# phylovi/libsbn

Hardware: AMD Instinct MI355X
Metric: tree log-likelihoods+gradients/sec (batched) (higher is better)
Workload: dtype f64; 1 GPU; DS1 27 taxa x 934 site patterns x 1000 trees per step over 1 GPU(s), JC69+weibull+4 (K=4), phylo_gradients: logL + branch + site gradients; trees_total=1000, trees_per_gpu=1000, taxa=27, patterns=934, categories=4, parallelism=single GPU

## Files before the change

### libsbn_amd/csrc/kernels_walk3.hip

```cpp
#include <hip/hip_runtime.h>

#include <algorithm>
#include <cmath>
#include <cstdlib>
#include <string>
#include <type_traits>

#include "mi_phylo_device_utils.h"
#include "mi_phylo_kernels.h"
#include "mi_phylo_setup_device.h"

namespace miphylo {
namespace {
using namespace dev;

template <int SHIFT>
__device__ __forceinline__ double row_shr_add(double v) {
  const int lo = __double2loint(v), hi = __double2hiint(v);
  const int slo = __builtin_amdgcn_update_dpp(0, lo, 0x110 + SHIFT, 0xf, 0xf, true);
  const int shi = __builtin_amdgcn_update_dpp(0, hi, 0x110 + SHIFT, 0xf, 0xf, true);
  return v + __hiloint2double(shi, slo);
}
template <int SHIFT>
__device__ __forceinline__ double row_ror_add(double v) {
// ... 1022 lines not shown
        store16_sc1(dst + 48, v4i32{me.gslot[1], me.gslot[2], me.gslot[3], me.pad});
      }
    }
  }
  asm volatile("s_waitcnt lgkmcnt(0)" ::: "memory");
  if (ok) {
    if (q == 0) {
      double* dst = reinterpret_cast<double*>(f.ms.models + t);
      const double* src = reinterpret_cast<const double*>(md);
      static_assert(sizeof(DevModel) % 16 == 0, "whole 16-byte pieces");
      for (int i = lane; i < (int)(sizeof(DevModel) / 16); i += 64) store16_sc1(dst + 2 * i, src[2 * i], src[2 * i + 1]);
    }
    const int idx = q * per_q + lane;
    const int node = idx / K, k = idx - node * K;
    const bool live = lane < per_q && node < N - 1;
    if (live) {
      double bl;
      if (!a.rooted) {
        bl = node < N - 2 ? a.bl[(size_t)t * (N - 1) + node] : 0.0;
      } else {
        bl = a.bl[(size_t)t * N + node];
        if (a.rates) bl *= a.rates[(size_t)t * (N - 1) + node];
      }
      const bool tip = node < n;
      lut_record(*md, md->cat_rate[k] * bl, tip, stage + lane * 41);
      const int slot = slot_of[node], m = slot / 6, pos = slot - m * 6;
      const int rec8 = (int)((((size_t)t * max_macros(n) + m) * 6 + pos) * (kPos / 8));
      rec_of[lane] = rec8 + k * (tip ? (int)(kTipCat / 8) : 32);
      len_of[lane] = tip ? 40 : 32;
    } else {
      rec_of[lane] = -1;
      len_of[lane] = 0;
    }
    asm volatile("s_waitcnt lgkmcnt(0)" ::: "memory");
    XSTAMP(st3);
    {
      int rec[8], len[8];
      double va[24], vb[24];
      const int part = lane & 7;
#pragma unroll
      for (int x8 = 0; x8 < 8; x8++) {
        const int th = (lane >> 3) + 8 * x8;
        rec[x8] = rec_of[th];
        len[x8] = len_of[th];
        const int row = min(th, per_q - 1) * 41;
#pragma unroll
        for (int p3 = 0; p3 < 3; p3++) {
          const int d = 2 * (p3 * 8 + part);
          va[3 * x8 + p3] = stage[row + min(d, 38)];
          vb[3 * x8 + p3] = stage[row + min(d, 38) + 1];
        }
      }
#pragma unroll
      for (int i = 0; i < 24; i++) asm volatile("" : "+v"(va[i]), "+v"(vb[i]));
#pragma unroll
      for (int x8 = 0; x8 < 8; x8++)
#pragma unroll
        for (int p3 = 0; p3 < 3; p3++) {
          const int d = 2 * (p3 * 8 + part);
          if (rec[x8] >= 0 && d < len[x8])
            store16_sc1(f.mmats + (size_t)rec[x8] + d, va[3 * x8 + p3], vb[3 * x8 + p3]);
        }
    }
  }
  XSTAMP(st4);
  asm volatile("s_waitcnt vmcnt(0)" ::: "memory");
  XSTAMP(st5);
#ifdef W3_SETUP_STAMPS
  if (lane == 0 && (t == 0 || t == 60 || t == 124) && q < 2)
    printf("setup role t %d q %d: start %lld end %lld model %lld tree %lld records %lld stores issued %lld landed %lld (10 ns ticks)\n", t, q, st0, (long long)__builtin_amdgcn_s_memrealtime(),
           st1 - st0, st2 - st1, st3 - st2, st4 - st3, st5 - st4);
#endif
  if (f.fence == 2) __builtin_amdgcn_fence(__ATOMIC_RELEASE, "agent");
  if (lane == 0 && f.ready && !(f.debug_skip == t + 1 && q == 1))
    __hip_atomic_fetch_add(f.ready + (size_t)t * kReadyStride, kReadyQuarter + (q == 0 ? M : 0), __ATOMIC_RELAXED,
                           __HIP_MEMORY_SCOPE_AGENT);
}

__global__ __launch_bounds__(kTile) void setup_records_kernel(FusedSetupArgs f) {
  extern __shared__ double wlds[];
  fused_setup_role(f, blockIdx.x, reinterpret_cast<char*>(wlds));
}

template <bool RESCALE, int KP>
__global__ __launch_bounds__(kTile, kRegs == 2 ? 3 : 2) void gradient_walk_lut_fused_kernel(LikArgs a, FusedSetupArgs f) {
  extern __shared__ double wlds[];
  if ((int)blockIdx.x < f.setup_blocks) {
    fused_setup_role(f, blockIdx.x, reinterpret_cast<char*>(wlds));
    return;
  }
  walk_lut_body<RESCALE, true, false, KP>(a, wlds, (int)blockIdx.x - f.setup_blocks, f.ready, f.spin_ticks, f.fence);
#ifdef W3_SETUP_STAMPS
  if (threadIdx.x == 0 && (((int)blockIdx.x - f.setup_blocks) % 1499) == 0)
    printf("walk block %d: out %lld\n", (int)blockIdx.x - f.setup_blocks, (long long)__builtin_amdgcn_s_memrealtime());
#endif
}

}

size_t gradient_walk_lut_mats_bytes_per_eval(int n) { return (size_t)max_macros(n) * kVisit; }

static int lut_kp(int K) { return K == 1 ? 1 : (K == 2 ? 2 : 4); }

bool gradient_walk_lut_fused_applies(int n, int K) {
  return gradient_walk_lut_applies(K) && 2 * n - 1 <= 64 && ((2 * n - 2) * K + 3) / 4 <= 64;
}

template <bool RESCALE, int KP>
static void launch_fused_variant(const LikArgs& a, const FusedSetupArgs& f, dim3 grid, size_t lds, hipStream_t s) {
  allow_large_lds(reinterpret_cast<const void*>(gradient_walk_lut_fused_kernel<RESCALE, KP>), lds);
  hipLaunchKernelGGL((gradient_walk_lut_fused_kernel<RESCALE, KP>), grid, dim3(kTile), lds, s, a, f);
}
void launch_gradient_walk_lut_fused(const LikArgs& a_in, const FusedSetupArgs& f_in, int count, bool rescale,
                                    hipStream_t s) {
  if (count <= 0) return;
  LikArgs a = a_in;
  FusedSetupArgs f = f_in;
  a.kp = lut_kp(a.K);
  a.cat_groups = 1;
  a.walk_evals = count;
  f.setup_blocks = kSetupQuarters * count;
  f.xcd_base = f.setup_blocks & 7;
  if (f.spin_ticks <= 0) f.spin_ticks = 100 * 1000 * 1000;
  const int gtiles = gradient_mfma_tiles(a.P, a.K);
  const dim3 grid((unsigned)((size_t)count * gtiles + f.setup_blocks));
  const size_t lds = std::max<size_t>(gradient_walk_lds_bytes(a.n, a.K, rescale, false), fused_setup_lds(a.n, a.K));
  switch ((rescale ? 8 : 0) | a.kp) {
    case 1: launch_fused_variant<false, 1>(a, f, grid, lds, s); break;
    case 2: launch_fused_variant<false, 2>(a, f, grid, lds, s); break;
    case 4: launch_fused_variant<false, 4>(a, f, grid, lds, s); break;
    case 9: launch_fused_variant<true, 1>(a, f, grid, lds, s); break;
    case 10: launch_fused_variant<true, 2>(a, f, grid, lds, s); break;
    default: launch_fused_variant<true, 4>(a, f, grid, lds, s); break;
  }
}

void launch_setup_records(const FusedSetupArgs& f_in, int count, hipStream_t s) {
  if (count <= 0) return;
  FusedSetupArgs f = f_in;
  f.setup_blocks = kSetupQuarters * count;
  f.xcd_base = 0;
  f.ready = nullptr;
  f.fence = 0;
  f.debug_skip = 0;
  const size_t lds = fused_setup_lds(f.ts.n, f.ms.K);
  allow_large_lds(reinterpret_cast<const void*>(setup_records_kernel), lds);
  hipLaunchKernelGGL(setup_records_kernel, dim3((unsigned)f.setup_blocks), dim3(kTile), lds, s, f);
}

void launch_transition_lut(const TransitionMacroArgs& a, hipStream_t s) {
  if (a.count <= 0) return;
  const int per_eval = (a.N - 1) * a.K;
  const dim3 grid(a.count, (per_eval + kTlBlock - 1) / kTlBlock);
  hipLaunchKernelGGL(transition_lut_kernel, grid, dim3(kTlBlock), sizeof(int) * (size_t)(a.N - 1), s, a);
}

bool gradient_walk_lut_applies(int K) { return K >= 1 && K <= 4 && kRegs >= 2; }

template <bool RESCALE, bool ARENA, int KP, int RR>
static void launch_lut_variant(const LikArgs& a, dim3 grid, size_t lds, hipStream_t s, bool resident,
                               int forced) {
  if (ARENA && (forced < 0 ? (a.g_tiles * RR <= 48 * kRegs || resident) : forced != 0)) {
    allow_large_lds(reinterpret_cast<const void*>(gradient_walk_lut_kernel<RESCALE, ARENA, KP, ARENA, RR>), lds);
    hipLaunchKernelGGL((gradient_walk_lut_kernel<RESCALE, ARENA, KP, ARENA, RR>), grid, dim3(kTile), lds, s, a);
    return;
  }
  allow_large_lds(reinterpret_cast<const void*>(gradient_walk_lut_kernel<RESCALE, ARENA, KP, false, RR>), lds);
  hipLaunchKernelGGL((gradient_walk_lut_kernel<RESCALE, ARENA, KP, false, RR>), grid, dim3(kTile), lds, s, a);
}
template <bool ARENA, int RR = kRegs>
static void launch_lut_store(const LikArgs& a, dim3 grid, size_t lds, bool rescale, hipStream_t s,
                             int arena_nt, bool resident = false) {
  switch ((rescale ? 8 : 0) | a.kp) {
    case 1: launch_lut_variant<false, ARENA, 1, RR>(a, grid, lds, s, resident, arena_nt); break;
    case 2: launch_lut_variant<false, ARENA, 2, RR>(a, grid, lds, s, resident, arena_nt); break;
    case 4: launch_lut_variant<false, ARENA, 4, RR>(a, grid, lds, s, resident, arena_nt); break;
    case 9: launch_lut_variant<true, ARENA, 1, RR>(a, grid, lds, s, resident, arena_nt); break;
    case 10: launch_lut_variant<true, ARENA, 2, RR>(a, grid, lds, s, resident, arena_nt); break;
    default: launch_lut_variant<true, ARENA, 4, RR>(a, grid, lds, s, resident, arena_nt); break;
  }
}

void launch_gradient_walk_lut(const LikArgs& a_in, int count, bool rescale, const Switches& sw, hipStream_t s) {
  if (count <= 0) return;
  LikArgs a = a_in;
  a.kp = lut_kp(a.K);
  a.cat_groups = 1;
  a.walk_evals = count;
  const bool wide = kRegs < kRegsWide && a.tile_regs == kRegsWide;
  const int regs = wide ? kRegsWide : kRegs;
  const int gtiles = gradient_mfma_tiles(a.P, a.K, regs);
  const bool arena_variant =
      a.store ? a.store == 2
              : gradient_walk_use_arena(sw.gradient_store, a.n, a.K, rescale, false, (size_t)gtiles * (size_t)count, true, regs);
  const dim3 grid((unsigned)((size_t)count * gtiles));
  if (arena_variant) {
    const int usual = gradient_arena_slots_usual(a.n), sure = gradient_arena_slots_sure(a.n);
    auto lds_for = [&](int slots) { return gradient_walk_lds_bytes_for(a.n, a.K, rescale, false, slots, regs); };
    auto launch = [&](int slots, bool resident) {
      if (wide) launch_lut_store<true, kRegsWide>(a, grid, lds_for(slots), rescale, s, sw.arena_nt, resident);
      else launch_lut_store<true>(a, grid, lds_for(slots), rescale, s, sw.arena_nt, resident);
    };
    a.lds_lo = -1;
    if (arena_single_launch(lds_for(sure), grid.x)) {
      a.lds_slots = sure;
      launch(sure, true);
      return;
    }
    a.lds_slots = usual;
    const bool resident = arena_single_launch(lds_for(usual), grid.x);
    launch(usual, resident);
    if (sure > usual) {
      a.lds_lo = usual;
      a.lds_slots = sure;
      launch(sure, resident);
    }
    return;
  }
  if (wide) {
    const size_t lds = gradient_walk_lds_bytes(a.n, a.K, rescale, false, regs);
    auto go = [&](auto kernel) {
      allow_large_lds(reinterpret_cast<const void*>(kernel), lds);
      hipLaunchKernelGGL(kernel, grid, dim3(kTile), lds, s, a);
    };
    switch ((rescale ? 8 : 0) | a.kp) {
      case 1: go(gradient_walk_lut_kernel<false, false, 1, false, kRegsWide, 1>); break;
      case 2: go(gradient_walk_lut_kernel<false, false, 2, false, kRegsWide, 1>); break;
      case 4: go(gradient_walk_lut_kernel<false, false, 4, false, kRegsWide, 1>); break;
      case 9: go(gradient_walk_lut_kernel<true, false, 1, false, kRegsWide, 1>); break;
      case 10: go(gradient_walk_lut_kernel<true, false, 2, false, kRegsWide, 1>); break;
// ... 38 lines not shown
```

### libsbn_amd/csrc/mi_phylo_call.cpp

```cpp
#include "mi_phylo_engine.h"

namespace {

bool use_arena(const mi_engine* e, bool rescale, bool subst, size_t waves = (size_t)-1, int regs = 0) {
  const bool lut = walk3_possible(e) && e->sw.walk3_arena && !subst && gradient_mfma_groups(e->K) == 1;
  return gradient_walk_use_arena(e->sw.gradient_store, e->n, e->K, rescale, subst, waves, lut, regs);
}
bool walk_fits(const mi_engine* e, bool rescale) { return gradient_walk_fits(e->n, e->K, rescale); }

const char* loglik_kernel_of(const mi_engine* e, bool rescaling) {
  LikArgs probe{};
  probe.n = e->n;
  probe.K = e->K;
  probe.tip_masks = e->have_tip_masks ? e->tip_masks.as<uint8_t>() : nullptr;
  return loglik_kernel_name(probe, rescaling, e->max_slots, e->sw);
}
bool matrix_core_gradient(const mi_engine* e, bool rescaling, bool loglik_is_valu) {
  return !e->sw.hbm_gradient && e->have_tip_masks && walk_fits(e, rescaling) &&
         reduce_tiles_fits(e->N) && (gradient_mfma_groups(e->K) == 1 || !loglik_is_valu);
}

size_t plv_bytes_per_eval(const mi_engine* e) {
  return (size_t)(e->n - 1) * e->K * e->tiles * kTile * 4 * sizeof(double);
}
// ... 38 lines not shown
  const int n = e->n;
  const bool gradient = kind == kGradientCall;
  p.kind = kind;
  p.T = T;
  p.rescaling = rescaling;
  p.rooted = rooted;
  p.gtr = e->spec.subst_model == MI_SUBST_GTR;
  p.groups = 1;
  p.models_per_tree = 1;
  p.E = p.M = T;
  p.mmats_bytes_per_eval = std::max(gradient_walk_mats_bytes_per_eval(n, e->K),
                                    walk3_possible(e) ? gradient_walk_lut_mats_bytes_per_eval(n) : 0);
  p.dominant = loglik_kernel_of(e, rescaling);
  p.loglik_is_valu = std::string(p.dominant) == "loglik_onchip_kernel";
  if (kind == kHessianCall) {
    p.Eg = T;
    p.mfma = !e->sw.hbm_gradient && e->have_tip_masks && e->K <= 4 && walk_fits(e, rescaling);
    p.g_tiles = p.mfma ? gradient_mfma_tiles(e->P, e->K) : e->tiles;
    const size_t waves = (size_t)(route_T ? route_T : T) * gradient_mfma_tiles(e->P, e->K);
    const bool arena = p.mfma && gradient_walk_use_arena(e->sw.gradient_store, n, e->K, rescaling, false, waves, false, 0);
    p.store = !p.mfma ? kStoreHbm : arena ? kStoreArena : kStoreLds;
    p.reserve_arena = arena;
    p.need_slots = !p.mfma;
    p.dominant = p.mfma ? gradient_walk_hess_kernel_name() : gradient_hessian_kernel_name();
    return p;
  }
  if (kind == kNniCall) {
    p.Eg = T;
    p.g_tiles = e->tiles;
    p.store = kStoreHbm;
    p.dominant = nni_scan_kernel_name();
    return p;
  }
  if (kind == kAncestralCall) {
    p.Eg = T;
    p.g_tiles = e->tiles;
    p.store = kStoreHbm;
    p.dominant = ancestral_kernel_name();
    return p;
  }
  if (kind == kPlacementCall) {
    p.Eg = T;
    p.g_tiles = e->tiles;
    p.store = kStoreHbm;
    p.dominant = placement_kernel_name();
    return p;
  }
  if (kind == kSprCall) {
    p.Eg = T;
    p.g_tiles = e->tiles;
    p.store = kStoreHbm;
    p.dominant = spr_kernel_name();
    return p;
  }
  p.mfma = gradient && matrix_core_gradient(e, rescaling, p.loglik_is_valu);
  if (p.mfma) p.groups = gradient_mfma_groups(e->K);
  p.analytic = e->sw.analytic_subst && p.mfma && p.gtr;
  p.tile_regs = p.mfma && !p.analytic && p.groups == 1 ? e->tile_regs : 0;
  p.g_tiles = p.mfma ? gradient_mfma_tiles(e->P, e->K, p.tile_regs) * p.groups : e->tiles;
  p.light = gradient && p.mfma && !p.analytic && p.gtr && !want_subst && !want_site;
  const bool fd = gradient && p.gtr && !p.analytic && !p.light;
  p.site_fused = gradient && e->K > 1 && !fd;
  p.site_separate = gradient && e->K > 1 && fd;
  p.models_per_tree = fd ? kFdModels : 1;
  p.M = T * p.models_per_tree;
  p.Eg = gradient ? T : 0;
  if (fd) p.E += 16 * T;
  if (p.site_separate) {
    p.E += T;
    p.Eg += T;
  }
  p.need_slots = !(gradient && p.mfma && p.groups == 1 && (!p.gtr || p.analytic || p.light));
  const bool arena = p.mfma && use_arena(e, rescaling, p.analytic, (size_t)T * (size_t)p.g_tiles, p.tile_regs);
  p.store = !p.mfma ? kStoreHbm : arena ? kStoreArena : kStoreLds;
  p.reserve_arena = p.mfma && (e->tile_regs || use_arena(e, false, true) || use_arena(e, true, true) ||
                               use_arena(e, false, false) || use_arena(e, true, false));
  p.hand_off_words = gradient && e->fused_setup && walk3_possible(e);
  const bool fuse_possible = p.mfma && walk3_possible(e) && !p.analytic && p.groups == 1 && !arena && !p.tile_regs && e->fused_setup &&
                             e->sw.fuse_finalize && p.E == T && p.models_per_tree == 1 && !p.need_slots &&
                             T <= e->sw.fused_max_trees && gradient_walk_lut_fused_applies(n, e->K);
  p.walk3 = p.mfma && walk3_possible(e) && !p.analytic && p.groups == 1 &&
            (p.tile_regs || (arena ? e->sw.walk3_arena : (e->K > 1 || e->sw.walk3_k1_lds || fuse_possible)));
  p.fuse_setup = p.walk3 && fuse_possible;
  p.setup_records = p.walk3 && !p.fuse_setup && !arena && !p.tile_regs && !p.analytic && p.groups == 1 && e->fused_setup &&
                    p.E == T && p.models_per_tree == 1 && !p.need_slots && T <= kMaxEvals &&
                    gradient_walk_lut_fused_applies(n, e->K) && e->sw.setup_records;
  p.fd_pass = gradient && p.gtr && !p.analytic && want_subst;
  p.site_pass = p.site_separate && want_site;
  p.loglik_runs = !gradient || p.fd_pass || (p.mfma && p.groups > 1);
  p.need_tip_tables = p.loglik_runs && p.loglik_is_valu;
  if (gradient)
    p.dominant = p.fuse_setup ? gradient_walk_lut_fused_kernel_name()
                 : p.walk3    ? gradient_walk_lut_kernel_name()
                 : p.mfma     ? gradient_walk_kernel_name()
                              : gradient_kernel_name();
  return p;
}

std::string plan_path(const mi_engine* e, const CallPlan& p) {
  std::string path = p.dominant;
  if (p.kind != kLogLikCall)
    path += p.store == kStoreHbm ? " store=hbm" : (p.store == kStoreArena ? " store=arena" : " store=lds");
  path += p.fuse_setup ? " setup=in-walk" : (p.setup_records ? " setup=with-records" : " setup=own-launch");
  if (p.kind == kHessianCall) path += " hess";
  if (p.kind == kNniCall) path += " nni";
  if (p.kind == kAncestralCall) path += " ancestral";
  if (p.kind == kPlacementCall) path += " placement";
  if (p.kind == kSprCall) path += " spr";
  if (p.pattern_ll) path += " pattern_ll";
  if (p.tile_regs > kLlR) path += " tile=wide";
  if (p.fd_pass) path += " fd=16";
  if (p.site_pass) path += " site-pass";
  if (p.light) path += " light";
  if (p.analytic) path += " analytic";
  if (p.rescaling) path += " rescaled";
  if (p.rooted) path += " rooted";
  return path + " K=" + std::to_string(e->K);
}

int reserve(mi_engine* e, const CallPlan& p) {
  const int n = e->n, N = e->N, T = p.T;
  const bool gradient = p.kind == kGradientCall;
  if (e->tree_scratch.ensure(sizeof(int32_t) * (size_t)T * 13 * N)) return 1;
  if (e->sched.ensure(sizeof(SchedEntry) * (size_t)T * (n - 1))) return 1;
  if (e->macros.ensure(sizeof(MacroEntry) * (size_t)T * macro_stride(n))) return 1;
  if (e->macro_count.ensure(sizeof(int32_t) * (size_t)T)) return 1;
  if (e->bl_eff.ensure(sizeof(double) * (size_t)T * N)) return 1;
  if (e->models.ensure(sizeof(DevModel) * (size_t)p.M)) return 1;
  if (e->mats.ensure(sizeof(double) * (size_t)p.E * (N - 1) * e->K * 16)) return 1;
  if (e->tip_tables.ensure(sizeof(double) * (size_t)p.E * n * e->K * 20)) return 1;
  if (gradient) {
    if (e->mmats.ensure(p.mmats_bytes_per_eval * (size_t)p.Eg)) return 1;
    if (p.analytic && e->mphi.ensure(p.mmats_bytes_per_eval / 2 * (size_t)p.Eg)) return 1;
  }
  if (p.analytic && e->x_sum.ensure(sizeof(double) * (size_t)p.Eg * kSubstExtra)) return 1;
  if (e->ll_part.ensure(sizeof(double) * (size_t)p.E * e->ll_stride)) return 1;
  if (e->fin_scratch.ensure(sizeof(double) * (size_t)T * 6 * n)) return 1;
  if (e->status.ensure(sizeof(int32_t) * kStatusWords)) return 1;
  if (p.hand_off_words && e->ready.bytes < sizeof(int32_t) * kReadyStride * (size_t)T) {
    if (e->ready.ensure(sizeof(int32_t) * kReadyStride * (size_t)T)) return 1;
    HIP_TRY(hipMemset(e->ready.ptr, 0, e->ready.bytes));
    HIP_TRY(hipDeviceSynchronize());
  }
  if (e->ll_sum.ensure(sizeof(double) * (size_t)p.E)) return 1;
  if (p.kind == kLogLikCall && !p.rooted && e->pattern_ll_out.ensure(sizeof(double) * (size_t)T)) return 1;
  if (gradient && e->g_sum.ensure(sizeof(double) * (size_t)p.Eg * 2 * N)) return 1;
  if (gradient) {
    const size_t per = plv_bytes_per_eval(e);
    const size_t chunk = std::max<size_t>(1, std::min<size_t>(p.Eg, e->plv_budget / per));
    if (!p.mfma && e->plv.ensure(per * chunk)) return 1;
    if (p.reserve_arena) {
      const size_t aper = gradient_arena_bytes_per_eval(n, e->P, e->K);
      const size_t achunk = std::max<size_t>(1, std::min<size_t>(p.Eg, e->plv_budget / aper));
      if (e->plv.ensure(aper * achunk)) return 1;
      if (e->arena_macros.ensure(sizeof(MacroEntry) * (size_t)T * macro_stride(n))) return 1;
      if (e->slot_need.ensure(sizeof(int32_t) * (size_t)T)) return 1;
    }
    const size_t g_width = std::max<size_t>(2 * (size_t)N, (size_t)gradient_mfma_width(n, true));
    if (e->g_part.ensure(sizeof(double) * (size_t)p.Eg * e->ll_stride * gradient_mfma_groups(e->K) *
                         g_width))
      return 1;
    if (e->site_lik.ensure(sizeof(double) * (size_t)p.Eg * e->tiles * kTile)) return 1;
    if (e->site_exp.ensure(sizeof(int32_t) * (size_t)p.Eg * e->tiles * kTile)) return 1;
  }
  return 0;
}


TreeSetupArgs tree_setup_args(const mi_engine* e, const DeviceCall& d, const CallPlan& p) {
  TreeSetupArgs ts{};
  ts.n = e->n;
  ts.T = d.T;
  ts.rooted = d.rooted;
  ts.parent_ids = d.parent_ids;
  ts.bl = d.bl;
  ts.rates = (d.rooted && (d.gradient || d.with_jacobian)) ? d.rates : nullptr;
  ts.scratch = e->tree_scratch.as<int32_t>();
  ts.sched = e->sched.as<SchedEntry>();
  ts.macros = p.mfma ? e->macros.as<MacroEntry>() : nullptr;
  ts.macro_count = e->macro_count.as<int32_t>();
  ts.bl_eff = e->bl_eff.as<double>();
  ts.status = e->status.as<int32_t>();
  ts.max_slots = e->max_slots;
  ts.need_slots = p.need_slots;
  ts.arena_macros = p.store == kStoreArena ? e->arena_macros.as<MacroEntry>() : nullptr;
  ts.slot_need = e->slot_need.as<int32_t>();
// ... 113 lines not shown
  la.map = EvalMap{d.T, p.models_per_tree};
  la.models = e->models.as<DevModel>();
  la.sched = e->sched.as<SchedEntry>();
  la.macros = walk_macros(e, p);
  la.macro_count = e->macro_count.as<int32_t>();
  la.mats = e->mats.as<double>();
  la.mmats = e->mmats.as<double>();
  la.tip_states = e->tip_states.as<int8_t>();
  la.tip_masks = e->have_tip_masks ? e->tip_masks.as<uint8_t>() : nullptr;
  la.tip_partials = e->spec.use_tip_states ? nullptr : e->tip_partials.as<double>();
  la.weights = e->weights.as<double>();
  la.ll_part = e->ll_part.as<double>();
  la.plv = e->plv.as<double>();
  la.g_part = e->g_part.as<double>();
  la.status = e->status.as<int32_t>();
  la.slot_need = e->slot_need.as<int32_t>();
  la.store = p.store;
  if (p.kind == kAncestralCall) {
    la.anc_state = d.out_anc_state;
    la.anc_map = d.out_anc_map;
    la.anc_cat = d.out_anc_cat;
    la.anc_rate = d.out_anc_rate;
    la.anc_tip = d.out_anc_tip;
    return la;
  }
  if (p.kind == kPlacementCall) {
    la.place_half = e->place_half.as<double>();
    la.place_pend = e->place_pend.as<double>();
    la.place_table = e->place_table.as<double>();
    la.place_G = d.G;
    return la;
  }
  if (p.kind == kHessianCall || p.kind == kNniCall || p.kind == kSprCall) return la;
  la.tip_tables = e->tip_tables.as<double>();
  la.mphi = e->mphi.as<double>();
  la.tip_code_tiles = e->have_tip_codes && e->tip_code_tiles.ptr && e->sw.tip_tiles && e->tile_regs == p.tile_regs
                          ? e->tip_code_tiles.as<uint8_t>() : nullptr;
  la.tip_tiles = e->have_tip_masks && e->tip_tiles.ptr && e->sw.tip_tiles ? e->tip_tiles.as<uint8_t>() : nullptr;
  la.tip_codes = e->have_tip_codes ? e->tip_codes.as<uint8_t>() : nullptr;
  la.tile_regs = p.tile_regs;
  la.pattern_ll = p.pattern_ll ? d.out_pattern_ll : nullptr;
  la.pattern_blank = e->pattern_blank.as<uint8_t>();
  return la;
}

void macro_slots(const mi_engine* e, int T, hipStream_t s) {
  launch_macro_slots(e->macros.as<MacroEntry>(), e->arena_macros.as<MacroEntry>(),
                     e->macro_count.as<int32_t>(), e->n, T, e->slot_need.as<int32_t>(),
                     e->status.as<int32_t>(), e->sw, s);
}

void note_call(mi_engine* e, const CallPlan& p, int first_launch_evals, int walk_launches) {
  e->dominant = p.dominant;
  e->last_path = plan_path(e, p);
  e->prof_first_launch_evals = first_launch_evals;
  e->last_evals = p.E;
  e->last_grad_evals = p.Eg;
  e->last_walk_launches = walk_launches;
}

int check_call(const mi_engine* e, const DeviceCall& d, const void* output) {
  if (d.T <= 0) return fail("tree_count must be positive");
  if (!d.parent_ids || !d.bl || !output) return fail("null tree / output pointer");
  if (e->param_count > 0 && !d.params) return fail("null parameter matrix");
  return 0;
}

}

int run_device(mi_engine* e, hipStream_t s, const DeviceCall& d_in) {
  HIP_TRY(hipSetDevice(e->spec.device));
  if (e->s == kAa) return d_in.out_pattern_ll ? fail(kPatternLl4State) : aa_run_device(e, s, d_in);
  if (check_call(e, d_in, d_in.out_pattern_ll ? d_in.out_pattern_ll : d_in.out_ll)) return 1;
  const CallPlan p = plan_call(e, d_in.gradient ? kGradientCall : kLogLikCall, d_in);
  if (reserve(e, p)) return 1;
  DeviceCall d = d_in;
  if (!d.out_ll) d.out_ll = e->pattern_ll_out.as<double>();
  const int n = e->n, N = e->N, T = d.T;
  const bool prof = e->prof_used < e->prof_capacity;
  const bool marks = prof && e->prof_phases;
  PROF_MARK(e, marks, 0, s);

  if (p.setup_records) launch_setup_records(fused_setup_args(e, d, p), T, s);
  const bool slots_done = !p.fuse_setup && !p.setup_records &&
                          launch_setup(tree_setup_args(e, d, p), model_setup_args(e, d, p), e->sw, s);
  if (p.store == kStoreArena && !slots_done) macro_slots(e, T, s);

  TransitionArgs tr = transition_args(e, d, p);
  if (p.mfma && p.groups == 1) {
    if (p.fd_pass) {
      tr.eval_base = T;
      tr.E = 16 * T;
      launch_transition(tr, s);
    }
  } else {
    launch_transition(tr, s);
  }
  auto macro_matrices = [&](int eval_begin, int grad_begin, int count) {
    const TransitionMacroArgs tm = transition_macro_args(e, d, p, eval_begin, grad_begin, count);
    if (p.walk3) launch_transition_lut(tm, s);
    else launch_transition_macro(tm, s);
  };
  if (p.mfma && !p.fuse_setup && !p.setup_records) {
    macro_matrices(0, 0, T);
    if (p.site_pass) macro_matrices(17 * T, T, T);
  }

  const LikArgs la = lik_args(e, d, p);
  int walk_launches = 0;
  auto loglik_range = [&](int eval_begin, int count) {
    launch_in_parts(e, count, 0, walk_launches, [&](int done, int part) {
      LikArgs l = la;
      l.eval_offset = eval_begin + done;
      launch_loglik(l, part, d.rescaling, e->max_slots, e->sw, s);
    });
  };
  auto grad_range = [&](int eval_begin, int grad_begin, int count) {
    launch_in_parts(e, count, vector_bytes_per_eval(e, p), walk_launches, [&](int done, int part) {
      LikArgs g = la;
      g.eval_offset = eval_begin + done;
      g.grad_offset = grad_begin + done;
      if (!p.mfma) return launch_gradient_hbm(g, part, d.rescaling, s);
      if (p.groups > 1) {
        g.site_lik = e->site_lik.as<double>();
        g.site_exp = e->site_exp.as<int32_t>();
        launch_loglik(g, part, d.rescaling, e->max_slots, e->sw, s);
      }
      if (p.fuse_setup) launch_gradient_walk_lut_fused(g, fused_setup_args(e, d, p), part, d.rescaling, s);
      else if (p.walk3) launch_gradient_walk_lut(g, part, d.rescaling, e->sw, s);
      else launch_gradient_walk(g, part, d.rescaling, p.analytic, e->sw, s);
    });
  };
  if (prof) HIP_TRY(hipEventRecord(prof_event(e, 0), s));
  PROF_MARK(e, marks, 1, s);
  PROF_MARK(e, marks, 2, s);
  if (!d.gradient) {
    loglik_range(0, T);
    if (prof) HIP_TRY(hipEventRecord(prof_event(e, 1), s));
    PROF_MARK(e, marks, 3, s);
  } else {
    grad_range(0, 0, T);
    if (prof) HIP_TRY(hipEventRecord(prof_event(e, 1), s));
    PROF_MARK(e, marks, 3, s);
    if (p.fd_pass) loglik_range(T, 16 * T);
    if (p.site_pass) grad_range(17 * T, T, T);
  }
  note_call(e, p, T, walk_launches);

  FinalizeArgs fa = finalize_args(e, d);
  fa.ll_tiles = e->ll_stride;
  fa.g_tiles = p.g_tiles;
  fa.ll_part = e->ll_part.as<double>();
  fa.g_part = e->g_part.as<double>();
  const int ll_kernel_count = p.loglik_is_valu ? e->tiles : loglik_mfma_tiles(e->P, e->K);
  const int grad_kernel_count =
      p.mfma ? (p.groups > 1 ? ll_kernel_count : p.g_tiles) : e->tiles;
  LlCounts ll_used{d.gradient ? grad_kernel_count : ll_kernel_count, ll_kernel_count, 0, 0};
  if (d.gradient && p.gtr && !p.analytic && !p.light) {
    ll_used.mid_lo = T;
    ll_used.mid_hi = 17 * T;
  }
  fa.ll_used = ll_used;
  bool fused = false;
  ReduceArgs ra{};
  if (reduce_tiles_fits(N)) {
    ra.N = N;
    ra.E = p.E;
    ra.Eg = p.Eg;
    ra.ll_tiles = e->ll_stride;
    ra.ll_used = ll_used;
    ra.g_tiles = p.g_tiles;
    ra.ll_part = e->ll_part.as<double>();
    ra.g_part = e->g_part.as<double>();
    ra.ll_sum = e->ll_sum.as<double>();
    ra.g_sum = e->g_sum.as<double>();
    ra.g_width = p.mfma ? gradient_mfma_width(n, p.analytic) : 0;
    ra.extra = p.analytic ? kSubstExtra : 0;
    ra.x_sum = e->x_sum.as<double>();
    ra.n = n;
    ra.T = T;
    ra.macros = walk_macros(e, p);
    ra.macro_count = e->macro_count.as<int32_t>();
    fused = e->sw.fuse_finalize && p.E == T;
    if (!fused) launch_reduce_tiles(ra, s);
    fa.ll_tiles = 1;
    fa.ll_used = LlCounts{1, 1, 0, 0};
// ... 405 lines not shown
```

### libsbn_amd/csrc/mi_phylo_engine.h

```cpp
#pragma once
#include <hip/hip_runtime.h>

#include <algorithm>
#include <cstring>
#include <functional>
#include <string>
#include <vector>

#include "../../include/mi_phylo.h"
#include "mi_phylo_host_arrays.h"
#include "mi_phylo_kernels.h"

namespace miphylo {
int fail(const std::string& msg);
void set_last_error(const std::string& msg);
}
using miphylo::fail;
using namespace miphylo;

#define HIP_TRY(expr)                                                              \
  do {                                                                             \
    hipError_t err__ = (expr);                                                     \
    if (err__ != hipSuccess)                                                       \
      return fail(std::string("HIP error: ") + hipGetErrorString(err__) + " at " + \
// ... 118 lines not shown
  int fused_fallbacks = 0;
  Buffer aa_model, aa_matP, aa_matPT, aa_tipP, aa_tipPQ, aa_exp_cum, aa_exp_loc,
      aa_root_val, aa_root_exp, aa_root_scale;
  bool aa_reserved_gradient = false;
  PinnedArena pinned;
  Switches sw;
  int tile_regs = 0;
  std::vector<mi_engine*> shards;
  int shard_mode = 0;
  std::vector<double> shard_sums;
  Buffer red_ll, red_g, red_site, red_sort;
  long red_ws_entries = -1;
  int red_ws_bits = 0;
  size_t red_ws_bytes = 0;
  Buffer in_pack, out_pack;
  Buffer opt_ws;
  int32_t* opt_word = nullptr;
  Buffer nni_apply_ws;
  Buffer nni_search_ws;
  Buffer pattern_blank;
  Buffer pattern_ll_out;
  Buffer rell_ws;
  Buffer rell_s;
  Buffer dist_codes;
  Buffer dist_model;
  Buffer dist_counts;
  Buffer dist_matrix;
  Buffer nj_ws;
  Buffer place_bl;
  Buffer place_half;
  Buffer place_pend;
  Buffer place_table;
  Buffer spr_bl;
  Buffer spr_half;
  Buffer spr_ws;
  Buffer spr_path;
  Buffer spr_apply_ws;
  Buffer spr_search_ws;
  Buffer split_ws;
  Buffer split_store;
  Buffer split_sort;
  Buffer rf_ws;
  size_t plv_budget = (size_t)8 << 30;
  std::vector<hipEvent_t> prof_events;
  int prof_capacity = 0, prof_used = 0;
  bool prof_phases = false;
  int prof_first_launch_evals = 0;
  const char* dominant = "";
  std::string last_path;
  int64_t last_evals = 0, last_grad_evals = 0;
  int status_tree_offset = 0;
  int last_walk_launches = 1;
  int aa_backoffs = 0;
};


constexpr int kProfEvents = 7;
inline hipEvent_t prof_event(mi_engine* e, int which) {
  return e->prof_events[(size_t)kProfEvents * e->prof_used + which];
}
#define PROF_MARK(e, on, which, s)                                   \
  do {                                                               \
    if (on) HIP_TRY(hipEventRecord(prof_event(e, 2 + (which)), s)); \
  } while (0)

enum CallKind { kLogLikCall, kGradientCall, kHessianCall, kNniCall, kAncestralCall, kPlacementCall, kSprCall };
enum WalkStore { kStoreHbm = 0, kStoreLds = 1, kStoreArena = 2 };
struct CallPlan {
  CallKind kind;
  int T;
  bool rescaling, rooted;
  int E, Eg, M, models_per_tree;
  bool gtr, site_fused, site_separate;
  bool mfma;
  bool walk3;
  WalkStore store;
  int groups;
  int tile_regs;
  int g_tiles;
  bool analytic;
  bool light;
  bool fuse_setup;
  bool setup_records;
  bool need_slots;
  bool fd_pass, site_pass;
  bool loglik_runs;
  bool loglik_is_valu;
  bool pattern_ll;
  bool need_tip_tables;
  size_t mmats_bytes_per_eval;
  bool reserve_arena;
  bool hand_off_words;
  const char* dominant;
};
struct DeviceCall {
  bool gradient = false, rooted = false, with_jacobian = false, rescaling = false;
  int T = 0;
  const int32_t* parent_ids = nullptr;
  const double* bl = nullptr;
  const double* params = nullptr;
  const double* rates = nullptr;
  const int32_t* rate_counts = nullptr;
  const double* heights = nullptr;
  const double* bounds = nullptr;
  const double* ratios = nullptr;
  double* out_ll = nullptr;
  double* out_branch = nullptr;
  double* out_ratios = nullptr;
  double* out_clock = nullptr;
  double* out_site = nullptr;
  double* out_subst = nullptr;
  double* out_hess = nullptr;
  double* out_gsq = nullptr;
  double* out_nni = nullptr;
  int32_t* out_best = nullptr;
  double* out_pattern_ll = nullptr;
  double* out_anc_state = nullptr;
  int8_t* out_anc_map = nullptr;
  double* out_anc_cat = nullptr;
  double* out_anc_rate = nullptr;
  double* out_anc_tip = nullptr;
  int Q = 0, C = 0, G = 0;
  const int8_t* query_states = nullptr;
  const int32_t* column_pattern = nullptr;
  const double* column_weights = nullptr;
  const double* pendant_lengths = nullptr;
  double* out_place_edge_ll = nullptr;
  int8_t* out_place_pendant = nullptr;
  int32_t* out_place_best = nullptr;
  double* out_place_lwr = nullptr;
  double* out_place_tables = nullptr;
  int spr_radius = 0;
  int32_t* out_spr_target = nullptr;
  double* out_spr_delta = nullptr;
  int32_t* out_spr_move = nullptr;
  double* out_spr_table = nullptr;
  int route_T = 0;
};
CallPlan plan_call(const mi_engine* e, CallKind kind, int T, bool rescaling, int route_T = 0,
                   bool rooted = false, bool want_site = true, bool want_subst = true);
inline CallPlan plan_call(const mi_engine* e, CallKind kind, const DeviceCall& d) {
  CallPlan p = plan_call(e, kind, d.T, d.rescaling, d.route_T, d.rooted, d.out_site != nullptr, d.out_subst != nullptr);
  p.pattern_ll = kind == kLogLikCall && d.out_pattern_ll != nullptr;
  return p;
}
std::string plan_path(const mi_engine* e, const CallPlan& p);
bool walk3_possible(const mi_engine* e);
int engine_tile_regs(const mi_engine* e);
int reserve(mi_engine* e, const CallPlan& p);
int reserve_hessian(mi_engine* e, const CallPlan& p);
int reserve_hessian_calls(mi_engine* e, int T);
TreeSetupArgs tree_setup_args(const mi_engine* e, const DeviceCall& d, const CallPlan& p);
ModelSetupArgs model_setup_args(const mi_engine* e, const DeviceCall& d, const CallPlan& p);
FinalizeArgs finalize_args(const mi_engine* e, const DeviceCall& d);
int run_device(mi_engine* e, hipStream_t s, const DeviceCall& d);
int run_hessian_device(mi_engine* e, hipStream_t s, const DeviceCall& d);
int reserve_nni_calls(mi_engine* e, int T);
int run_nni_device(mi_engine* e, hipStream_t s, const DeviceCall& d);
int reserve_ancestral_calls(mi_engine* e, int T);
int run_ancestral_device(mi_engine* e, hipStream_t s, const DeviceCall& d);
int check_placement_shape(const mi_engine* e, int Q, int C, int G);
int reserve_placement_calls(mi_engine* e, int T, int G);
int run_placement_device(mi_engine* e, hipStream_t s, const DeviceCall& d);
int check_spr_shape(const mi_engine* e, int radius);
int reserve_spr_calls(mi_engine* e, int T);
int run_spr_device(mi_engine* e, hipStream_t s, const DeviceCall& d);
// ... 102 lines not shown
```

### libsbn_amd/csrc/mi_phylo_kernels.h

```cpp
#pragma once
#include <hip/hip_runtime.h>

#include "mi_phylo_device.h"
#include "mi_phylo_switches.h"

namespace miphylo {

struct EvalMap {
  int T;
  int models_per_tree;
  __host__ __device__ void decode(int e, int& tree, int& model) const {
    if (e < T) {
      tree = e;
      model = e * models_per_tree;
    } else if (e < 17 * T) {
      tree = (e - T) / 16;
      model = tree * kFdModels + 1 + (e - T) % 16;
    } else {
      tree = e - 17 * T;
      model = tree * kFdModels + 16;
    }
  }
};

// ... 446 lines not shown
}
struct SplitArgs {
  int n, T, W, capacity;
  int hash_bits;
  uint32_t slots;
  const int32_t* parent_ids;
  const double* bl;
  const double* weights;
  int32_t* status;
  uint32_t* store;
  uint32_t* occ_bits;
  uint64_t* occ_hash;
  int32_t* occ_slot;
  void* scan_tmp;
  size_t scan_tmp_bytes;
  int32_t* slot_owner;
  int32_t* slot_first;
  int32_t* slot_trees;
  uint32_t *keys, *vals, *keys2, *vals2;
  void* sort_tmp;
  size_t sort_tmp_bytes;
  int32_t* out_index;
  int32_t* out_count;
  uint32_t* out_bits;
  int32_t* out_first;
  int32_t* out_trees;
  double* out_stats;
};
size_t split_scan_tmp_bytes(size_t occurrences);
size_t split_sort_tmp_bytes(size_t occurrences);
int launch_split_index(const SplitArgs& a, hipStream_t s);
struct RfArgs {
  int n, T;
  const int32_t* split_index;
  const double* bl;
  int32_t* sorted_index;
  double* sorted_length;
  int32_t* sorted_count;
  int32_t* out_rf;
  double* out_bs;
};
void launch_rf(const RfArgs& a, hipStream_t s);
int gradient_mfma_groups(int K);
int gradient_mfma_width(int n, bool subst = false);
void launch_macro_slots(const MacroEntry* macros_in, MacroEntry* macros_out,
                        const int32_t* macro_count, int n, int T, int32_t* need, int32_t* status,
                        const Switches& sw, hipStream_t s);
size_t gradient_arena_bytes_per_eval(int n, int P, int K);
int device_compute_units();
bool arena_single_launch(size_t lds_bytes, size_t waves);
int gradient_arena_slots_sure(int n);
int gradient_arena_slots_usual(int n);
void launch_transition_macro(const TransitionMacroArgs& a, hipStream_t s);
void launch_gradient_walk(const LikArgs& a, int count, bool rescale, bool subst, const Switches& sw, hipStream_t s);
bool gradient_walk_fits(int n, int K, bool rescale);
bool gradient_walk_use_arena(int store, int n, int K, bool rescale, bool subst, size_t waves = (size_t)-1,
                             bool lut = false, int regs = 0);
bool gradient_walk_batches_take_arena(int n, int K, bool lut);
size_t gradient_walk_lds_bytes(int n, int K, bool rescale, bool subst, int regs = 0);
size_t gradient_walk_lds_bytes_for(int n, int K, bool rescale, bool subst, int slots, int regs = 0);
size_t gradient_walk_mats_bytes_per_eval(int n, int K);
const char* gradient_walk_kernel_name();
size_t gradient_walk_lut_mats_bytes_per_eval(int n);
void launch_transition_lut(const TransitionMacroArgs& a, hipStream_t s);
bool gradient_walk_lut_applies(int K);
void launch_gradient_walk_lut(const LikArgs& a, int count, bool rescale, const Switches& sw, hipStream_t s);
constexpr int kReadyStride = 32;
struct FusedSetupArgs {
  TreeSetupArgs ts;
  ModelSetupArgs ms;
  double* mmats;
  int32_t* ready;
  int setup_blocks;
  int spin_ticks;
  int debug_skip;
  int fence;
  int colocate;
  int xcd_base;
};
bool gradient_walk_lut_fused_applies(int n, int K);
void launch_gradient_walk_lut_fused(const LikArgs& a, const FusedSetupArgs& f, int count, bool rescale,
                                    hipStream_t s);
void launch_setup_records(const FusedSetupArgs& f, int count, hipStream_t s);
const char* gradient_walk_lut_kernel_name();
const char* gradient_walk_lut_fused_kernel_name();
int gradient_walk_waves_per_cu(int store, int n, int K);
struct ReduceArgs {
  int N, E, Eg, ll_tiles, g_tiles;
  LlCounts ll_used;
  const double* ll_part;
  const double* g_part;
  double* ll_sum;
  double* g_sum;
  int g_width, n, T;
  const MacroEntry* macros;
  const int32_t* macro_count;
  int extra;
  double* x_sum;
  int keep_offset;
};

struct SubstGradArgs {
  int T, param_count, rates_off, freqs_off;
  const double* params;
  const DevModel* models;
  const double* x_sum;
  double* out_subst;
};
void launch_subst_gradient(const SubstGradArgs& a, hipStream_t s);
constexpr int kSubstExtra = 68;
struct ViReduceArgs {
  int T, N, index_count;
  const double* ll;
  const double* branch;
  const double* site;
  const int32_t* branch_index;
  const double* tree_weights;
  double* out_sums;
  double* out_index_gradient;
};
size_t vi_reduce_workspace_bytes(long entries, int index_count);
int launch_vi_reduce(const ViReduceArgs& a, void* workspace, size_t workspace_bytes, hipStream_t s);
bool reduce_tiles_fits(int N);
void launch_reduce_tiles(const ReduceArgs& a, hipStream_t s);
void launch_finalize(const FinalizeArgs& a, hipStream_t s);
void launch_reduce_finalize(const ReduceArgs& ra, const FinalizeArgs& fa, hipStream_t s);

constexpr int kAa = 20;
constexpr int kAaTile = 16;
constexpr int kAaTipSlack = 512;
constexpr int kAaTileDoubles = 320;
constexpr int kAaPack = 512;
constexpr int kAaPackRows16 = 320;
constexpr int kAaTipTable = 21 * 20;
constexpr int kAaPreTiles = 2;

struct AaModel {
  double pi[kAa];
  double lambda[kAa];
  double Q[kAa * kAa];
  double V[kAa * kAa];
  double Vinv[kAa * kAa];
  double Qpack[kAaPack];
};

struct AaTransitionArgs {
  int n, N, K;
  int eval_offset, evals;
  int gradient;
  const AaModel* model;
  const DevModel* models;
  const double* bl_eff;
  double* matP;
  double* matPT;
  double* tipP;
  double* tipPQ;
};

struct AaWalkArgs {
  int n, N, P, K;
  int tiles;
  int eval_offset, evals;
  int gradient;
  int slots;
  int ring_slots;
  int pre_ring_slots;
// ... 42 lines not shown
```

### libsbn_amd/csrc/mi_phylo_switches.cpp

```cpp
#include "mi_phylo_switches.h"

#include <cerrno>
#include <climits>
#include <cstdlib>
#include <cstring>

namespace miphylo {
namespace {

struct Reader {
  std::string error;

  const char* get(const char* name) {
    const char* v = getenv(name);
    return v && *v ? v : nullptr;
  }
  void reject(const char* name, const char* value, const std::string& expected) {
    if (error.empty()) error = std::string(name) + "=" + value + ": expected " + expected;
  }
  int choice(const char* name, const char* values, int dflt) {
    const char* v = get(name);
    if (!v) return dflt;
    const size_t len = strlen(v);
    int index = 0;
    for (const char* w = values;; index++) {
      const char* end = strchr(w, '|');
      const size_t wlen = end ? (size_t)(end - w) : strlen(w);
      if (wlen == len && strncmp(w, v, len) == 0) return index;
      if (!end) break;
      w = end + 1;
    }
    reject(name, v, values);
    return dflt;
  }
  bool on_off(const char* name, bool dflt) { return choice(name, "0|1", dflt ? 1 : 0) == 1; }
  int listed(const char* name, const char* values, int dflt) {
    return choice(name, values, -1) < 0 ? dflt : atoi(get(name));
  }
  long long integer(const char* name, long long lo, long long hi, long long dflt) {
    const char* v = get(name);
    if (!v) return dflt;
    char* end = nullptr;
    errno = 0;
    const long long x = strtoll(v, &end, 10);
    if (end != v && *end == '\0' && errno == 0 && x >= lo && x <= hi) return x;
    reject(name, v, hi == LLONG_MAX ? "an integer >= " + std::to_string(lo)
                                    : "an integer in [" + std::to_string(lo) + ", " + std::to_string(hi) + "]");
    return dflt;
  }
  double number(const char* name, double lo, double hi, const char* range, double dflt) {
    const char* v = get(name);
    if (!v) return dflt;
    char* end = nullptr;
    errno = 0;
    const double x = strtod(v, &end);
    if (end != v && *end == '\0' && errno == 0 && x >= lo && x <= hi) return x;
    reject(name, v, std::string("a number in ") + range);
    return dflt;
  }
};

}

bool parse_switches(Switches& out, std::string& error) {
  Reader r;
  Switches s;
  s.hbm_gradient = r.choice("MI_PHYLO_GRADIENT_PATH", "mfma|hbm", 0) == 1;
  s.walk3 = r.choice("MI_PHYLO_GRADIENT_WALK", "v2|v3", 1) == 1;
  s.walk3_arena = r.on_off("MI_PHYLO_WALK3_ARENA", true);
  s.walk3_k1_lds = r.on_off("MI_PHYLO_WALK3_K1", true);
  s.gradient_store = r.choice("MI_PHYLO_GRADIENT_STORE", "lds|arena", -1) + 1;
  s.walk_tile_regs = r.listed("MI_PHYLO_WALK_TILE_REGS", "3|4", 0);
  s.walk_tiles_per_wave = (int)r.integer("MI_PHYLO_WALK_TILES_PER_WAVE", 1, INT_MAX, 0);
  s.arena_nt = r.listed("MI_PHYLO_ARENA_NT", "0|1", -1);
  s.tip_tiles = r.on_off("MI_PHYLO_TIP_TILES", true);
  s.analytic_subst = r.choice("MI_PHYLO_SUBST_GRADIENT", "fd|analytic", 0) == 1;
  s.loglik_path = r.choice("MI_PHYLO_LOGLIK_PATH", "valu|mfma", -1) + 1;
  s.loglik_evals_per_wave = r.listed("MI_PHYLO_LOGLIK_EVALS_PER_WAVE", "1|2|4|8", 0);
  s.tree_setup = r.choice("MI_PHYLO_TREE_SETUP", "small|wg|lds", -1) + 1;
  s.macro_slots = r.choice("MI_PHYLO_MACRO_SLOTS", "own|seq", -1) + 1;
  s.setup_records = r.on_off("MI_PHYLO_SETUP_RECORDS", false);
  s.fused_setup = r.on_off("MI_PHYLO_FUSED_SETUP", true);
  s.fuse_finalize = r.on_off("MI_PHYLO_FUSE_FINALIZE", true);
  s.fused_max_trees = (int)r.integer("MI_PHYLO_FUSED_MAX_TREES", 0, INT_MAX, 512);
  s.fused_fence = r.choice("MI_PHYLO_FUSED_FENCE", "none|l1|agent", 1);
  s.fused_colocate = r.on_off("MI_PHYLO_FUSED_COLOCATE", true);
  s.fused_spin_ticks = (int)(r.number("MI_PHYLO_FUSED_SPIN_MS", 0.01, 2.0e4, "[0.01, 20000]", 0.0) * 1.0e5);
  s.fused_debug_skip = (int)r.integer("MI_PHYLO_DEBUG_FUSED_SKIP", 0, INT_MAX, 0);
  s.plv_bytes = r.integer("MI_PHYLO_PLV_BYTES", 0, LLONG_MAX, -1);
  s.place_table_global = r.choice("MI_PHYLO_PLACE_TABLE", "lds|global", 0) == 1;
  s.split_hash_bits = (int)r.integer("MI_PHYLO_SPLIT_HASH_BITS", 0, 32, 32);
  s.aa_jacobi_seq = r.choice("MI_PHYLO_AA_JACOBI", "wave|seq", 0) == 1;
  s.aa_post_wave = r.choice("MI_PHYLO_AA_POST", "wg|wave", 0) == 1;
  s.aa_pre_wave = r.choice("MI_PHYLO_AA_PRE", "wg|wave", 0) == 1;
  s.aa_post_tiles = r.listed("MI_PHYLO_AA_POST_TILES", "1|2|4", 0);
  s.aa_post_one_tile_below = (long)r.integer("MI_PHYLO_AA_POST_ONE_TILE_BELOW", 0, LONG_MAX, -1);
  s.aa_ring = r.listed("MI_PHYLO_AA_RING", "0|1|2|4", -1);
  s.aa_pre_ring = r.listed("MI_PHYLO_AA_PRE_RING", "0|1|2", -1);
  s.aa_lds_pad = (size_t)r.integer("MI_PHYLO_AA_LDS_PAD", 0, 160 * 1024, 0);
  error = r.error;
  if (!error.empty()) return false;
  out = s;
  return true;
}

}
```

### libsbn_amd/csrc/mi_phylo_switches.h

```cpp
#pragma once
#include <cstddef>
#include <string>

namespace miphylo {

struct Switches {
  bool hbm_gradient = false;
  bool walk3 = true;
  bool walk3_arena = true;
  bool walk3_k1_lds = true;
  int gradient_store = 0;
  int walk_tile_regs = 0;
  int walk_tiles_per_wave = 0;
  int arena_nt = -1;
  bool tip_tiles = true;
  bool analytic_subst = false;
  int loglik_path = 0;
  int loglik_evals_per_wave = 0;
  int tree_setup = 0;
  int macro_slots = 0;
  bool setup_records = false;
  bool fused_setup = true;
  bool fuse_finalize = true;
  int fused_max_trees = 512;
  int fused_fence = 1;
  bool fused_colocate = true;
  int fused_spin_ticks = 0;
  int fused_debug_skip = 0;
  long long plv_bytes = -1;
  bool place_table_global = false;
  int split_hash_bits = 32;
  bool aa_jacobi_seq = false;
  bool aa_post_wave = false;
  bool aa_pre_wave = false;
  int aa_post_tiles = 0;
  long aa_post_one_tile_below = -1;
  int aa_ring = -1;
  int aa_pre_ring = -1;
  size_t aa_lds_pad = 0;
};

bool parse_switches(Switches& out, std::string& error);

}
```

Measured before the change: 1.283 million trees/s.

## Add workgroup-per-tree setup kernel that builds tree, model and LUT records together

Adds a new setup kernel that uses one 4-wave workgroup per tree. Wave 0 builds the tree and wave 1 builds the model. All waves then compute transition LUT records, stage them through LDS and write them to global memory with coalesced 16-byte stores. The kernel replaces the separate tree/model setup and macro-matrix launches, and becomes the default when the walk is not fused (T=1000 exceeds the fused max of 512). The cost is a new code path with LDS staging and multiple passes that could be slower if occupancy or the serialized tree build dominates.

```diff
diff --git a/libsbn_amd/csrc/kernels_walk3.hip b/libsbn_amd/csrc/kernels_walk3.hip
--- a/libsbn_amd/csrc/kernels_walk3.hip
+++ b/libsbn_amd/csrc/kernels_walk3.hip
@@ -1128,6 +1128,131 @@
   fused_setup_role(f, blockIdx.x, reinterpret_cast<char*>(wlds));
 }
 
+constexpr int kSetupWgWaves = 4, kSetupWgThreads = 64 * kSetupWgWaves;
+constexpr unsigned kSetupWgLdsMax = 40u * 1024u;
+constexpr unsigned kSetupWgRowBytes = 41u * 8u;
+__host__ __device__ inline unsigned setup_wg_model_offset(int pass_rows) {
+  return (kSetupWgWaves * (unsigned)pass_rows * kSetupWgRowBytes + 127u) & ~127u;
+}
+__host__ __device__ inline unsigned setup_wg_lds(int pass_rows) {
+  return setup_wg_model_offset(pass_rows) + (unsigned)sizeof(DevModel) + 64u * 4u + 16u;
+}
+inline int setup_wg_pass_rows(int n, int K) {
+  const int per_q = ((2 * n - 2) * K + kSetupWgWaves - 1) / kSetupWgWaves;
+  for (int passes = 1;; passes++) {
+    const int h = (per_q + passes - 1) / passes;
+    if (setup_wg_lds(h) <= kSetupWgLdsMax || h == 1) return h;
+  }
+}
+
+template <bool JC>
+__global__ __launch_bounds__(kSetupWgThreads, JC ? 4 : 2) void setup_wg_kernel(FusedSetupArgs f, int pass_rows) {
+  extern __shared__ double wlds[];
+  char* lds = reinterpret_cast<char*>(wlds);
+  const TreeSetupArgs& a = f.ts;
+  const int t = blockIdx.x;
+  const int wave = __builtin_amdgcn_readfirstlane((int)threadIdx.x >> 6), lane = threadIdx.x & 63;
+  const int n = a.n, N = 2 * n - 1, K = f.ms.K;
+  const int per_q = ((N - 1) * K + kSetupWgWaves - 1) / kSetupWgWaves;
+  const int H = pass_rows;
+  double* stage = reinterpret_cast<double*>(lds) + wave * H * 41;
+  DevModel* md = reinterpret_cast<DevModel*>(lds + setup_wg_model_offset(H));
+  int* slot_of = reinterpret_cast<int*>(md + 1);
+  int* tree_ok = slot_of + 64;
+  static_assert(kSetupWgWaves * kSetupWgRowBytes >= kSmallTreeLdsInts * sizeof(int), "the tree build's scratch fits one staged row per wave");
+
+  const int idx = wave * per_q + lane;
+  const int node = idx / K, k = idx - node * K;
+  const bool live = lane < per_q && node < N - 1;
+  double bl = 0.0;
+  if (live) {
+    if (!a.rooted) {
+      bl = node < N - 2 ? a.bl[(size_t)t * (N - 1) + node] : 0.0;
+    } else {
+      bl = a.bl[(size_t)t * N + node];
+      if (a.rates) bl *= a.rates[(size_t)t * (N - 1) + node];
+    }
+  }
+
+  if (wave == 0) {
+    SmallTree<1> tree;
+    small_tree_build<1>(a, t, lane, tree, reinterpret_cast<int*>(lds));
+    const bool built = tree.status == kOk;
+    if (built && tree.is_macro[0]) {
+      const MacroEntry& me = tree.me[0];
+      const int base = tree.macro_rank[0] * 6;
+      slot_of[me.child[0]] = base;
+      slot_of[me.child[1]] = base + 1;
+#pragma unroll
+      for (int j = 0; j < 2; j++)
+        if (((me.shape >> (2 * j)) & 3) == 2) {
+          slot_of[me.grand[2 * j]] = base + 2 + 2 * j;
+          slot_of[me.grand[2 * j + 1]] = base + 3 + 2 * j;
+        }
+    }
+    if (lane == 0) *tree_ok = built ? 1 : 0;
+    small_tree_store<1>(a, t, lane, tree);
+  } else if (wave == 1) {
+    ModelSetupArgs ms = f.ms;
+    if (JC) ms.subst = 0;
+    model_setup_wave(ms, t, lane, *md);
+  }
+  __syncthreads();
+  if (!__builtin_amdgcn_readfirstlane(*tree_ok)) return;
+
+  if (wave == 1) {
+    dbl2* dst = reinterpret_cast<dbl2*>(f.ms.models + t);
+    const dbl2* src = reinterpret_cast<const dbl2*>(md);
+    static_assert(sizeof(DevModel) % 16 == 0, "whole 16-byte pieces");
+    for (int i = lane; i < (int)(sizeof(DevModel) / 16); i += 64) dst[i] = src[i];
+  }
+  double st[40];
+  int rec = -1, len = 0;
+  if (live) {
+    const bool tip = node < n;
+    lut_record(*md, md->cat_rate[k] * bl, tip, st);
+    const int slot = slot_of[node], m = slot / 6, pos = slot - m * 6;
+    const int rec8 = (int)((((size_t)t * max_macros(n) + m) * 6 + pos) * (kPos / 8));
+    rec = rec8 + k * (tip ? (int)(kTipCat / 8) : 32);
+    len = tip ? 40 : 32;
+  }
+  const int part = lane & 7;
+  for (int base = 0; base < per_q; base += H) {
+    if (live && lane >= base && lane < base + H) {
+      double* row = stage + (lane - base) * 41;
+#pragma unroll
+      for (int d = 0; d < 32; d++) row[d] = st[d];
+      if (len == 40) {
+#pragma unroll
+        for (int d = 32; d < 40; d++) row[d] = st[d];
+      }
+    }
+    asm volatile("s_waitcnt lgkmcnt(0)" ::: "memory");
+#pragma unroll
+    for (int x = 0; x < 4; x++) {
+      const int r = (lane >> 3) + 8 * x, owner = base + r;
+      const int rec_r = __shfl(rec, owner & 63, 64), len_r = __shfl(len, owner & 63, 64);
+      const bool have = r < H && owner < per_q && rec_r >= 0;
+      const double* row = stage + min(r, H - 1) * 41;
+      double va[3], vb[3];
+#pragma unroll
+      for (int p3 = 0; p3 < 3; p3++) {
+        const int d = 2 * (p3 * 8 + part);
+        va[p3] = row[min(d, 38)];
+        vb[p3] = row[min(d, 38) + 1];
+      }
+#pragma unroll
+      for (int p3 = 0; p3 < 3; p3++) asm volatile("" : "+v"(va[p3]), "+v"(vb[p3]));
+#pragma unroll
+      for (int p3 = 0; p3 < 3; p3++) {
+        const int d = 2 * (p3 * 8 + part);
+        if (have && d < len_r) *reinterpret_cast<dbl2*>(f.mmats + (size_t)rec_r + d) = dbl2{va[p3], vb[p3]};
+      }
+    }
+    asm volatile("s_waitcnt lgkmcnt(0)" ::: "memory");
+  }
+}
+
 template <bool RESCALE, int KP>
 __global__ __launch_bounds__(kTile, kRegs == 2 ? 3 : 2) void gradient_walk_lut_fused_kernel(LikArgs a, FusedSetupArgs f) {
   extern __shared__ double wlds[];
@@ -1192,6 +1317,20 @@
   const size_t lds = fused_setup_lds(f.ts.n, f.ms.K);
   allow_large_lds(reinterpret_cast<const void*>(setup_records_kernel), lds);
   hipLaunchKernelGGL(setup_records_kernel, dim3((unsigned)f.setup_blocks), dim3(kTile), lds, s, f);
+}
+
+void launch_setup_workgroups(const FusedSetupArgs& f_in, int count, hipStream_t s) {
+  if (count <= 0) return;
+  FusedSetupArgs f = f_in;
+  f.setup_blocks = count;
+  f.xcd_base = 0;
+  f.ready = nullptr;
+  f.fence = 0;
+  f.debug_skip = 0;
+  const int pass_rows = setup_wg_pass_rows(f.ts.n, f.ms.K);
+  const dim3 grid((unsigned)count), block(kSetupWgThreads);
+  if (f.ms.subst == 0) hipLaunchKernelGGL(setup_wg_kernel<true>, grid, block, setup_wg_lds(pass_rows), s, f, pass_rows);
+  else hipLaunchKernelGGL(setup_wg_kernel<false>, grid, block, setup_wg_lds(pass_rows), s, f, pass_rows);
 }
 
 void launch_transition_lut(const TransitionMacroArgs& a, hipStream_t s) {
diff --git a/libsbn_amd/csrc/mi_phylo_call.cpp b/libsbn_amd/csrc/mi_phylo_call.cpp
--- a/libsbn_amd/csrc/mi_phylo_call.cpp
+++ b/libsbn_amd/csrc/mi_phylo_call.cpp
@@ -144,9 +144,12 @@
   p.walk3 = p.mfma && walk3_possible(e) && !p.analytic && p.groups == 1 &&
             (p.tile_regs || (arena ? e->sw.walk3_arena : (e->K > 1 || e->sw.walk3_k1_lds || fuse_possible)));
   p.fuse_setup = p.walk3 && fuse_possible;
-  p.setup_records = p.walk3 && !p.fuse_setup && !arena && !p.tile_regs && !p.analytic && p.groups == 1 && e->fused_setup &&
-                    p.E == T && p.models_per_tree == 1 && !p.need_slots && T <= kMaxEvals &&
-                    gradient_walk_lut_fused_applies(n, e->K) && e->sw.setup_records;
+  const bool records_possible = p.walk3 && !p.fuse_setup && !arena && !p.tile_regs && !p.analytic && p.groups == 1 &&
+                                e->fused_setup && p.E == T && p.models_per_tree == 1 && !p.need_slots && T <= kMaxEvals &&
+                                gradient_walk_lut_fused_applies(n, e->K);
+  p.setup_records = records_possible && e->sw.setup_records == 1;
+  p.setup_wg = records_possible && (e->sw.setup_records == 2 ||
+                                    (e->sw.setup_records < 0 && e->sw.fuse_finalize && (e->N - 1) * e->K > 64));
   p.fd_pass = gradient && p.gtr && !p.analytic && want_subst;
   p.site_pass = p.site_separate && want_site;
   p.loglik_runs = !gradient || p.fd_pass || (p.mfma && p.groups > 1);
@@ -163,7 +166,10 @@
   std::string path = p.dominant;
   if (p.kind != kLogLikCall)
     path += p.store == kStoreHbm ? " store=hbm" : (p.store == kStoreArena ? " store=arena" : " store=lds");
-  path += p.fuse_setup ? " setup=in-walk" : (p.setup_records ? " setup=with-records" : " setup=own-launch");
+  path += p.fuse_setup      ? " setup=in-walk"
+          : p.setup_records ? " setup=with-records"
+          : p.setup_wg      ? " setup=workgroup-records"
+                            : " setup=own-launch";
   if (p.kind == kHessianCall) path += " hess";
   if (p.kind == kNniCall) path += " nni";
   if (p.kind == kAncestralCall) path += " ancestral";
@@ -443,7 +449,8 @@
   PROF_MARK(e, marks, 0, s);
 
   if (p.setup_records) launch_setup_records(fused_setup_args(e, d, p), T, s);
-  const bool slots_done = !p.fuse_setup && !p.setup_records &&
+  if (p.setup_wg) launch_setup_workgroups(fused_setup_args(e, d, p), T, s);
+  const bool slots_done = !p.fuse_setup && !p.setup_records && !p.setup_wg &&
                           launch_setup(tree_setup_args(e, d, p), model_setup_args(e, d, p), e->sw, s);
   if (p.store == kStoreArena && !slots_done) macro_slots(e, T, s);
 
@@ -462,7 +469,7 @@
     if (p.walk3) launch_transition_lut(tm, s);
     else launch_transition_macro(tm, s);
   };
-  if (p.mfma && !p.fuse_setup && !p.setup_records) {
+  if (p.mfma && !p.fuse_setup && !p.setup_records && !p.setup_wg) {
     macro_matrices(0, 0, T);
     if (p.site_pass) macro_matrices(17 * T, T, T);
   }
diff --git a/libsbn_amd/csrc/mi_phylo_engine.h b/libsbn_amd/csrc/mi_phylo_engine.h
--- a/libsbn_amd/csrc/mi_phylo_engine.h
+++ b/libsbn_amd/csrc/mi_phylo_engine.h
@@ -224,6 +224,7 @@
   bool light;
   bool fuse_setup;
   bool setup_records;
+  bool setup_wg;
   bool need_slots;
   bool fd_pass, site_pass;
   bool loglik_runs;
diff --git a/libsbn_amd/csrc/mi_phylo_kernels.h b/libsbn_amd/csrc/mi_phylo_kernels.h
--- a/libsbn_amd/csrc/mi_phylo_kernels.h
+++ b/libsbn_amd/csrc/mi_phylo_kernels.h
@@ -552,6 +552,7 @@
 void launch_gradient_walk_lut_fused(const LikArgs& a, const FusedSetupArgs& f, int count, bool rescale,
                                     hipStream_t s);
 void launch_setup_records(const FusedSetupArgs& f, int count, hipStream_t s);
+void launch_setup_workgroups(const FusedSetupArgs& f, int count, hipStream_t s);
 const char* gradient_walk_lut_kernel_name();
 const char* gradient_walk_lut_fused_kernel_name();
 int gradient_walk_waves_per_cu(int store, int n, int K);
diff --git a/libsbn_amd/csrc/mi_phylo_switches.cpp b/libsbn_amd/csrc/mi_phylo_switches.cpp
--- a/libsbn_amd/csrc/mi_phylo_switches.cpp
+++ b/libsbn_amd/csrc/mi_phylo_switches.cpp
@@ -79,7 +79,7 @@
   s.loglik_evals_per_wave = r.listed("MI_PHYLO_LOGLIK_EVALS_PER_WAVE", "1|2|4|8", 0);
   s.tree_setup = r.choice("MI_PHYLO_TREE_SETUP", "small|wg|lds", -1) + 1;
   s.macro_slots = r.choice("MI_PHYLO_MACRO_SLOTS", "own|seq", -1) + 1;
-  s.setup_records = r.on_off("MI_PHYLO_SETUP_RECORDS", false);
+  s.setup_records = r.choice("MI_PHYLO_SETUP_RECORDS", "0|1|wg", -1);
   s.fused_setup = r.on_off("MI_PHYLO_FUSED_SETUP", true);
   s.fuse_finalize = r.on_off("MI_PHYLO_FUSE_FINALIZE", true);
   s.fused_max_trees = (int)r.integer("MI_PHYLO_FUSED_MAX_TREES", 0, INT_MAX, 512);
diff --git a/libsbn_amd/csrc/mi_phylo_switches.h b/libsbn_amd/csrc/mi_phylo_switches.h
--- a/libsbn_amd/csrc/mi_phylo_switches.h
+++ b/libsbn_amd/csrc/mi_phylo_switches.h
@@ -19,7 +19,7 @@
   int loglik_evals_per_wave = 0;
   int tree_setup = 0;
   int macro_slots = 0;
-  bool setup_records = false;
+  int setup_records = -1;
   bool fused_setup = true;
   bool fuse_finalize = true;
   int fused_max_trees = 512;
```

Result: faster. 1.298 million trees/s (median of 6 runs) (+1.2%).
